# rahulaggarwal965/vslam

Measured on AMD Instinct MI355X. Metric: frame-pairs/sec (extract+match+RANSAC) @1280×720, 2k kp, 4096 hyp; 1/2/4/8 GPU, higher is better.
Workload: dtype u8/f32/f64; 1 GPU; C3: 1280x720, 2000 keypoints, 4096 hypotheses, batch 256 pairs per GPU, SURVEY 8(d) data: rotation + parallax, sub-pixel resampling, 40-45 % outlier matches; pairs_per_gpu=256, batches_in_flight=4

## Files before the change

vslam_amd/build.py:

```python
import os
import subprocess
import sys

HERE = os.path.dirname(os.path.abspath(__file__))
CSRC = os.path.join(HERE, "csrc")
LIB = os.path.join(HERE, "libvslam_amd.so")
SOURCES = ["capi.hip", "match.hip", "ransac_sets.hip", "ransac_solve.hip", "ransac_count.hip", "ransac_prune.hip", "ransac_select.hip", "refit.hip", "refine.hip",
           "kdtree.hip", "gray.hip", "response.hip", "select.hip", "blur.hip",
           "brief.hip", "orb_grid.hip", "pose.hip", "assoc.hip", "map.hip", "world.hip", "resect.hip", "adjust.hip", "render.hip", "multi.hip", "pipeline.hip"]
HEADERS = ["ctx.h", "introselect.h", "image_common.h", "ransac_svd.h", "ransac_residual.h", "ransac_prune_cert.h", "refine_math.h", "resect_math.h", "adjust_math.h", "world_select.h", "world_match.h",
           os.path.join("..", "..", "include", "vslam_amd.h"),
           os.path.join("..", "..", "include", "vslam_resect.h"),
           os.path.join("..", "..", "include", "vslam_adjust.h"),
           os.path.join("..", "..", "include", "vslam_brief_pattern_31.h")]
FLAGS = ["--offload-arch=gfx950", "-O3", "-std=c++17", "-ffp-contract=off", "-fPIC", "-Wall"]
EXTRA_FLAGS = {"response.hip": ["-fno-slp-vectorize"]}
OBJDIR = os.path.join(HERE, "_obj")


EXP_LIB = os.path.join(HERE, "libvslam_amd_exp.so")
EXP_OBJDIR = os.path.join(HERE, "_obj_exp")


def _compile(hipcc, src, verbose, objdir=None, extra=()):
    objdir = objdir or OBJDIR
    obj = os.path.join(objdir, src.replace(".hip", ".o"))
    deps = [os.path.join(CSRC, src)] + [os.path.join(CSRC, h) for h in HEADERS] + [os.path.abspath(__file__)]
    if os.path.exists(obj) and all(os.path.getmtime(d) <= os.path.getmtime(obj) for d in deps):
        return obj, None
    cmd = [hipcc] + FLAGS + list(extra) + EXTRA_FLAGS.get(src, []) + ["-c", "-o", obj, src]
    if verbose:
        print(" ".join(cmd))
    return obj, subprocess.Popen(cmd, cwd=CSRC)


def build(force=False, verbose=False, experiments=False):
    hipcc = os.environ.get("HIPCC", "/opt/rocm/bin/hipcc")
    objdir, lib, extra = (EXP_OBJDIR, EXP_LIB, ("-DVSLAM_EXPERIMENTS",)) if experiments else (OBJDIR, LIB, ())
    return _build(hipcc, objdir, lib, extra, force, verbose)


def _build(hipcc, OBJDIR, LIB, extra, force, verbose):
    os.makedirs(OBJDIR, exist_ok=True)
# ... 45 lines not shown
```

vslam_amd/capi.py:

```python
import ctypes as C
import os

_HERE = os.path.dirname(os.path.abspath(__file__))
LIB_PATH = os.environ.get("VSLAM_AMD_LIB") or os.path.join(_HERE, "libvslam_amd.so")
EXP_LIB_PATH = os.path.join(_HERE, "libvslam_amd_exp.so")

OK = 0
ERRORS = {-1: "VSLAM_ERR_INVALID", -2: "VSLAM_ERR_HIP", -3: "VSLAM_ERR_NO_DEVICE",
          -4: "VSLAM_ERR_CAPACITY", -5: "VSLAM_ERR_DEGENERATE", -6: "VSLAM_ERR_COMM"}

SYMBOLS = [
    "vslam_ctx_create", "vslam_ctx_make_current", "vslam_ctx_destroy", "vslam_ctx_set_stream", "vslam_ctx_set_option", "vslam_ctx_synchronize", "vslam_ctx_wait",
    "vslam_last_error", "vslam_ctx_workspace_bytes", "vslam_version", "vslam_brief_pattern_31", "vslam_dev_alloc", "vslam_dev_free", "vslam_copy_h2d",
    "vslam_copy_d2h", "vslam_debug_stream_copy", "vslam_debug_valu_calib", "vslam_prof_enable", "vslam_prof_reset", "vslam_prof_count", "vslam_prof_get",
    "vslam_match_knn2_ratio", "vslam_ransac_sets", "vslam_ransac_fundamental", "vslam_ransac_solve",
    "vslam_ransac_evaluate", "vslam_refit_fundamental", "vslam_refine_pairs", "vslam_kdtree_build",
    "vslam_kdtree_radius", "vslam_kdtree_nearest", "vslam_kdtree_cell_table", "vslam_extract_features", "vslam_extract_features_grid", "vslam_triangulate_points", "vslam_frontend_pairs_pose", "vslam_pipeline_batches_redone", "vslam_corner_stats", "vslam_bgr2gray", "vslam_min_eigen",
    "vslam_good_features", "vslam_gaussian7", "vslam_orb_describe", "vslam_extract_Rt", "vslam_triangulate", "vslam_associate_map_points", "vslam_reprojection_filter",
    "vslam_match_features",
    "vslam_map_create", "vslam_map_destroy", "vslam_map_reset", "vslam_map_step", "vslam_map_view", "vslam_map_observations",
    "vslam_track_sequences",
    "vslam_world_create", "vslam_world_destroy", "vslam_world_reset", "vslam_world_step", "vslam_world_lift", "vslam_world_view",
    "vslam_map_attach_world", "vslam_world_render",
    "vslam_view_default", "vslam_view_look_at", "vslam_render_points", "vslam_map_render",
# ... 218 lines not shown
        self._check(self.lib.vslam_prof_reset(self.handle))

    def prof_report(self):
        n = self.lib.vslam_prof_count(self.handle)
        if n < 0:
            self._check(n)
        out = {}
        for i in range(n):
            name = C.create_string_buffer(128)
            ms = C.c_double()
            cnt = C.c_int64()
            self._check(self.lib.vslam_prof_get(self.handle, C.c_int(i), name, C.c_int(128), C.byref(ms), C.byref(cnt)))
            out[name.value.decode()] = (ms.value, cnt.value)
        return out

    def debug_detect(self, bgr, max_corners, width=None):
        torch = self.torch
        F, H = bgr.shape[0], bgr.shape[1]
        W = width if width is not None else bgr.shape[2]
        stride = bgr.shape[2] * (bgr.shape[3] if bgr.dim() == 4 else 1)
        xy = torch.zeros((F, max_corners, 2), dtype=torch.float32, device=bgr.device)
        n = torch.zeros((F,), dtype=torch.int32, device=bgr.device)
        self._ready()
        self._check(self.lib.vslam_debug_detect(self.handle, _ptr(bgr), C.c_int(F), C.c_int(W), C.c_int(H), C.c_int(stride),
                                                C.c_int(max_corners), C.c_int(max_corners), _ptr(xy), _ptr(n)))
        return xy, n

    def debug_ransac_prune_x(self, batch, hyp):
        torch = self.torch
        x = torch.zeros((batch, hyp), dtype=torch.int32, device="cuda")
        self._ready()
        self._check(self.lib.vslam_debug_ransac_prune_x(self.handle, _ptr(x), C.c_int(batch), C.c_int(hyp)))
        return x

    def debug_ransac_prune_tile(self, F, xy):
        torch = self.torch
        self._dev(F, torch.float32, "F"); self._dev(xy, torch.float32, "xy")
        assert tuple(F.shape) == (32, 9) and tuple(xy.shape) == (4, 32)
        n = torch.zeros((32, 32), dtype=torch.float32, device=F.device)
        a0 = torch.zeros((32, 32), dtype=torch.float32, device=F.device)
        self._ready()
        self._check(self.lib.vslam_debug_ransac_prune_tile(self.handle, _ptr(F), _ptr(xy), _ptr(n), _ptr(a0)))
        return n, a0

    def debug_valu_calib(self):
        self._check(self.lib.vslam_debug_valu_calib(self.handle))

    def debug_stream_copy(self, src, dst, bytes_per_lane):
        self._check(self.lib.vslam_debug_stream_copy(self.handle, _ptr(src), _ptr(dst), C.c_size_t(src.numel() * src.element_size()),
                                                     C.c_int(bytes_per_lane)))

    def match_knn2_ratio(self, desc1, n1, desc2, n2, want_knn=False):
        torch = self.torch
        B, K, _ = desc1.shape
        self._dev(desc1, torch.uint8, "desc1"); self._dev(desc2, torch.uint8, "desc2")
        self._dev(n1, torch.int32, "n1"); self._dev(n2, torch.int32, "n2")
        pairs = torch.empty((B, K, 2), dtype=torch.int32, device=desc1.device)
        m = torch.empty((B,), dtype=torch.int32, device=desc1.device)
        knn = torch.empty((B, K, 4), dtype=torch.int32, device=desc1.device) if want_knn else None
        self._check(self.lib.vslam_match_knn2_ratio(self.handle, _ptr(desc1), _ptr(n1), _ptr(desc2), _ptr(n2),
                                                    C.c_int(B), C.c_int(K), _ptr(pairs), _ptr(m), _ptr(knn)))
        return (pairs, m, knn) if want_knn else (pairs, m)

    def ransac_sets(self, seeds, m, hyp):
        torch = self.torch
        B = seeds.shape[0]
# ... 937 lines not shown
```

vslam_amd/csrc/ransac_count.hip:

```cpp
#include "ransac_residual.h"

namespace {
using namespace vs_ransac;

constexpr int kCntHyps = 128;
constexpr int kCntWaves = 8;
constexpr int kCntQueue = 320;
constexpr int kCntLdsMatches = 4096;
constexpr int kScreenMatches = 128;
constexpr int kScreenHyps = 128;
constexpr int kRankThreads = 512;
constexpr int kPilotHyps = kRankThreads / 64;
constexpr int kCandMax = 8;
constexpr float kCntTinyDD = 0x1p-120f;
constexpr int kFcmpOGT = 2, kFcmpOLT = 4, kFcmpULT = 12;
constexpr int kCntRec = 12;
typedef __attribute__((address_space(3))) volatile uint32_t cnt_queue_t;
static_assert(VSLAM_MAX_KP <= 65536, "queue words keep the match index in 16 bits");

__host__ __device__ constexpr int cnt_pad(int n) { return (n + 255) & ~255; }
constexpr int kHeadUncertified = -1;
__device__ __forceinline__ float cnt_sum_rel(int adds) { return fmaxf(0x1p-18f, (float)(13 + adds) * 0x1p-24f); }

struct CntBand {
    float lo, hi;
    double beta;
    bool ok;
};
__device__ __forceinline__ CntBand cnt_band(const float *f, float C1, float C2, float threshold) {
    CntBand B;
    bool ok = threshold >= 0x1p-20f && threshold <= 0x1p20f && C1 <= 0x1p20f && C2 <= 0x1p20f;
#pragma unroll
// ... 384 lines not shown
            int p = __popcll(va & ~oa) + __popcll(vb & ~ob);
            int c = __popcll(va & ia) + __popcll(vb & ib);
            if (__builtin_amdgcn_fcmpf(fminf(dd[u].x, dd[u].y), kCntTinyDD, kFcmpULT) != 0ull) {
                p = n0;
                c = 0xFF;
            }
            mine = lane == j + u ? (p | (c << 8)) : mine;
            any_alive = any_alive || p + (m - n0) >= bound_pilots;
        }
        if (!any_alive) continue;
        float v[kU];
#pragma unroll
        for (int u = 0; u < kU; u++) v[u] = (in_a ? g[u].x : 0.f) + (in_b ? g[u].y : 0.f);
        const int z = 0;
        const float k01 = odd1 ? v[1] : v[0], t01 = odd1 ? v[0] : v[1], k23 = odd1 ? v[3] : v[2], t23 = odd1 ? v[2] : v[3];
        const float r01 = k01 + __int_as_float(__builtin_amdgcn_update_dpp(z, __float_as_int(t01), 0xB1, 0xF, 0xF, false));
        const float r23 = k23 + __int_as_float(__builtin_amdgcn_update_dpp(z, __float_as_int(t23), 0xB1, 0xF, 0xF, false));
        const float kk = odd2 ? r23 : r01, tt = odd2 ? r01 : r23;
        float r = kk + __int_as_float(__builtin_amdgcn_update_dpp(z, __float_as_int(tt), 0x4E, 0xF, 0xF, false));
        r += __int_as_float(__builtin_amdgcn_update_dpp(z, __float_as_int(r), 0x124, 0xF, 0xF, false));
        r += __int_as_float(__builtin_amdgcn_update_dpp(z, __float_as_int(r), 0x128, 0xF, 0xF, false));
        r += __shfl_xor(r, 16, 64);
        r += __shfl_xor(r, 32, 64);
        mine_sum = (lane >> 2) == (j >> 2) ? r : mine_sum;
    }
    const int h = hbase + wave * 32 + lane;
    if (lane < 32 && h < hyp) {
        const int c = mine >> 8;
        pot0[(size_t)b * hyp + h] = mine & 0xFF;
        head[(size_t)b * hyp + h] = make_int2(c == 0xFF ? kHeadUncertified : c, __float_as_int(mine_sum));
    }
}

__global__ __launch_bounds__(64 * kCandMax) void ransac_cand_kernel(
    const float *__restrict__ rk, int kp_pad, const int32_t *__restrict__ m_arr, int min_m, int kp_stride, int hyp,
    float threshold, const float *__restrict__ hypF, const int32_t *__restrict__ pot0, int by_sum,
    int32_t *__restrict__ cbound, unsigned long long *__restrict__ sfloor) {
    const int b = blockIdx.x, tid = threadIdx.x, lane = tid & 63;
    const int wave = __builtin_amdgcn_readfirstlane(tid >> 6);
    const int m = min(m_arr[b], kp_stride);
    if (m < min_m) return;
    __shared__ int s_max[kCandMax], s_l0[kCandMax][kCandMax], s_l1[kCandMax][kCandMax], s_n0[kCandMax], s_n1[kCandMax];
    __shared__ int s_cand[kCandMax], s_nc;
    const int32_t *P = pot0 + (size_t)b * hyp;
    int mx = -1;
    for (int i = tid; i < hyp; i += 64 * kCandMax) mx = max(mx, P[i]);
#pragma unroll
    for (int off = 32; off > 0; off >>= 1) mx = max(mx, __shfl_xor(mx, off, 64));
    if (lane == 0) s_max[wave] = mx;
    __syncthreads();
    mx = s_max[0];
    for (int w = 1; w < kCandMax; w++) mx = max(mx, s_max[w]);
    const int per = (hyp + kCandMax - 1) / kCandMax;
    const int lo = min(hyp, wave * per), hi = min(hyp, lo + per);
    int n0 = 0, n1 = 0;
    __shared__ int s_samp[kCandMax][32];
    int nsamp = 0;
    for (int i0 = lo; i0 < hi && ((by_sum && nsamp < 32) || n0 < kCandMax || n1 < kCandMax); i0 += 64) {
        const int i = i0 + lane;
        const int v = i < hi ? P[i] : -2;
        unsigned long long b0 = __ballot(v == mx), b1 = __ballot(v == mx - 1);
        if (by_sum) {
            const int rs = nsamp + __popcll(b0 & ((1ull << lane) - 1ull));
            if (v == mx && rs < 32) s_samp[wave][rs] = i;
            nsamp = min(32, nsamp + (int)__popcll(b0));
        }
        const int r0 = n0 + __popcll(b0 & ((1ull << lane) - 1ull)), r1 = n1 + __popcll(b1 & ((1ull << lane) - 1ull));
        if (v == mx && r0 < kCandMax) s_l0[wave][r0] = i;
        if (v == mx - 1 && r1 < kCandMax) s_l1[wave][r1] = i;
        n0 = min(kCandMax, n0 + __popcll(b0));
        n1 = min(kCandMax, n1 + __popcll(b1));
    }
    if (by_sum && nsamp > 1) {
        const int n128 = min(m, kScreenMatches);
        const float *r = rk + (size_t)b * 4 * kp_pad;
        const float2 x1 = *reinterpret_cast<const float2 *>(r + 2 * lane), y1 = *reinterpret_cast<const float2 *>(r + kp_pad + 2 * lane);
        const float2 x2 = *reinterpret_cast<const float2 *>(r + 2 * kp_pad + 2 * lane), y2 = *reinterpret_cast<const float2 *>(r + 3 * kp_pad + 2 * lane);
        v2f X1, Y1, X2, Y2;
        X1.x = x1.x; X1.y = x1.y; Y1.x = y1.x; Y1.y = y1.y;
        X2.x = x2.x; X2.y = x2.y; Y2.x = y2.x; Y2.y = y2.y;
        float fl[9];
        {
            const int hs = s_samp[wave][lane < nsamp ? lane : 0];
            const float *src = hypF + ((size_t)b * hyp + hs) * 9;
// ... 38 lines not shown
        s_nc = n;
    }
    __syncthreads();
    __shared__ int s_ccount[kCandMax];
    __shared__ double s_csum[kCandMax];
    if (wave < s_nc) {
        const int h = s_cand[wave];
        double esum = 0;
        const int count = cnt_exact_ranked(hypF + ((size_t)b * hyp + h) * 9, rk + (size_t)b * 4 * kp_pad, kp_pad, m, threshold, lane, &esum);
        if (lane == 0) {
            atomicMax(&cbound[b], count);
            s_ccount[wave] = count;
            s_csum[wave] = esum;
        }
    }
    __syncthreads();
    if (tid == 0) {
        int cb = -1;
        for (int k = 0; k < s_nc; k++) cb = max(cb, s_ccount[k]);
        double fl = -INFINITY;
        bool any_nan = false;
        for (int k = 0; k < s_nc; k++)
            if (s_ccount[k] == cb) {
                any_nan = any_nan || !(s_csum[k] == s_csum[k]);
                if (s_csum[k] > fl) fl = s_csum[k];
            }
        const bool valid = cb > 0 && !any_nan && fl > 0 && fl < 0x1p120;
        const float flf = (float)(fl * (1.0 - 0x1p-20));
        const unsigned long long mine = valid ? ((unsigned long long)(uint32_t)cb << 32) | (unsigned long long)__float_as_uint(flf) : 0ull;
        const unsigned long long pilots = sfloor[b];
        sfloor[b] = mine > pilots ? mine : pilots;
    }
}

#ifdef VSLAM_EXPERIMENTS
#define VS_CNT_PAYLOAD_PARAM , int exit_payload
#define VS_CNT_PAYLOAD_ARG , exit_payload
#else
#define VS_CNT_PAYLOAD_PARAM
#define VS_CNT_PAYLOAD_ARG
#endif
template <bool LDS, bool ZERO>
__global__ __launch_bounds__(64 * kCntWaves) __attribute__((amdgpu_waves_per_eu(6, 6))) void ransac_count_kernel(
    const float *__restrict__ rk, int kp_pad, const int32_t *__restrict__ m_arr, int min_m, int kp_stride, int hyp, float threshold,
    const float *__restrict__ hypF, const int32_t *__restrict__ pot0, const int2 *__restrict__ head,
    const float *__restrict__ cmax, int32_t *__restrict__ hyp_count, float *__restrict__ hyp_sum, float *__restrict__ approx,
    int32_t *__restrict__ cbound, const unsigned long long *__restrict__ sfloor VS_CNT_PAYLOAD_PARAM) {
    const int b = blockIdx.y, tid = threadIdx.x, lane = tid & 63;
    const int wave = __builtin_amdgcn_readfirstlane(tid >> 6);
    const int hbase = blockIdx.x * kCntHyps;
    const int nh = min(kCntHyps, hyp - hbase);
    const int m = min(m_arr[b], kp_stride);
    if (m < min_m) return;

    __shared__ __align__(16) float s_rec[kCntHyps * kCntRec];
    __shared__ int s_cnt[kCntHyps];
    __shared__ float s_part[kCntHyps];
    constexpr int kHeadMine = 0x10000, kHeadNoSum = 0x20000;
    __shared__ int s_unk[kCntHyps];
    __shared__ int s_state[kCntHyps];
    __shared__ int s_list[kCntHyps];
    constexpr int kListWaves = kCntHyps / 64;
    static_assert(kCntHyps % 64 == 0 && kListWaves <= kCntWaves, "whole waves find the survivors");
    __shared__ int s_nlist[kListWaves], s_next, s_bound;
    extern __shared__ __align__(16) uint32_t s_dyn[];

// ... 187 lines not shown
        if (st == 1 && my_ok && !s_unk[tid]) {
            const double Sd = (double)S;
            const double rel = (double)cnt_sum_rel(2 * ((m - (ZERO ? 0 : n0) + 255) >> 8) + 9);
            err = (float)((2.02 * my_beta * sqrt((double)m * Sd) + (double)m * my_beta * my_beta + rel * Sd) * (1.0 + 0x1p-20));
        }
        reinterpret_cast<float2 *>(approx)[out] = make_float2(S, err);
    }
}

}

int vs_launch_ransac_count(vslam_ctx *ctx, const float *xy1, const float *xy2, const int32_t *pairs, const int32_t *m,
                           const float *hypF, int batch, int kp_stride, int hyp, float threshold, int32_t *hyp_count,
                           float *hyp_sum, float *approx) {
    const int min_m = ctx->ransac_min_matches;
    int rc;
    int32_t *cbound = nullptr, *pot0 = nullptr;
    float *rk = nullptr, *cmax = nullptr;
    const int kp_pad = cnt_pad(kp_stride);
    if ((rc = vs_arena_get(ctx, "ransac.cbound", sizeof(int32_t) * (size_t)batch, (void **)&cbound))) return rc;
    unsigned long long *sfloor = nullptr;
    if ((rc = vs_arena_get(ctx, "ransac.sfloor", sizeof(unsigned long long) * (size_t)batch, (void **)&sfloor))) return rc;
    static const bool no_sum_rule = VS_EXPERIMENT_ENV("VSLAM_RANSAC_NO_SUM_RULE") != nullptr;
    const bool from_zero = VS_EXPERIMENT_ENV("VSLAM_RANSAC_COUNT_FROM_ZERO") != nullptr;
#ifdef VSLAM_EXPERIMENTS
    const int exit_payload = VS_EXPERIMENT_ENV("VSLAM_RANSAC_COUNT_EXIT_PAYLOAD") != nullptr ? 1 : 0;
#endif
    int2 *head = nullptr;
    if ((rc = vs_arena_get(ctx, "ransac.head", sizeof(int2) * (size_t)batch * hyp, (void **)&head))) return rc;
    const unsigned long long *use_floor = no_sum_rule ? nullptr : sfloor;
    if ((rc = vs_arena_get(ctx, "ransac.pot0", sizeof(int32_t) * (size_t)batch * hyp, (void **)&pot0))) return rc;
    if ((rc = vs_arena_get(ctx, "ransac.rk", sizeof(float) * 4 * (size_t)kp_pad * batch, (void **)&rk))) return rc;
    if ((rc = vs_arena_get(ctx, "ransac.cmax", sizeof(float) * 2 * (size_t)batch, (void **)&cmax))) return rc;
    {
        VsProfScope ps(ctx, "ransac_rank_kernel");
        ransac_rank_kernel<<<batch, kRankThreads, 0, ctx->stream>>>(xy1, xy2, pairs, m, min_m, kp_stride, kp_pad, hyp, threshold, hypF,
                                                                    cbound, rk, cmax, sfloor);
    }
    {
        VsProfScope ps(ctx, "ransac_screen_kernel");
        dim3 grid(vs_div_up(hyp, kScreenHyps), batch);
        ransac_screen_kernel<<<grid, 256, 0, ctx->stream>>>(rk, kp_pad, m, min_m, kp_stride, hyp, threshold, hypF, cmax, cbound, pot0, head);
    }
    {
        VsProfScope ps(ctx, "ransac_cand_kernel");
        ransac_cand_kernel<<<batch, 64 * kCandMax, 0, ctx->stream>>>(rk, kp_pad, m, min_m, kp_stride, hyp, threshold, hypF, pot0,
                                                                     no_sum_rule ? 0 : 1, cbound, sfloor);
    }
    if ((rc = vs_launch_ransac_prune(ctx, rk, kp_pad, m, min_m, kp_stride, hyp, threshold, hypF, cmax, cbound, pot0, batch, kScreenMatches)))
        return rc;
    if (int arc = vs_aux_job_point(ctx, 4)) return arc;
    {
        VsProfScope ps(ctx, "ransac_count_kernel");
        const bool lds = kp_pad <= kCntLdsMatches;
        const size_t dyn = (lds ? sizeof(float) * 4 * (size_t)kp_pad : 0) + sizeof(uint32_t) * kCntQueue * kCntWaves;
        const size_t dyn_max = sizeof(float) * 4 * kCntLdsMatches + sizeof(uint32_t) * kCntQueue * kCntWaves;
        dim3 grid(vs_div_up(hyp, kCntHyps), batch);
#ifdef VSLAM_EXPERIMENTS
        if (from_zero) {
            if (dyn > 32 * 1024 && (rc = vs_allow_dynamic_lds(ctx, ransac_count_kernel<true, true>, "ransac_count_from_zero", dyn_max)))
                return rc;
            if (lds)
                ransac_count_kernel<true, true><<<grid, 64 * kCntWaves, dyn, ctx->stream>>>(
                    rk, kp_pad, m, min_m, kp_stride, hyp, threshold, hypF, pot0, head, cmax, hyp_count, hyp_sum, approx, cbound,
                    use_floor VS_CNT_PAYLOAD_ARG);
            else
                ransac_count_kernel<false, true><<<grid, 64 * kCntWaves, dyn, ctx->stream>>>(
                    rk, kp_pad, m, min_m, kp_stride, hyp, threshold, hypF, pot0, head, cmax, hyp_count, hyp_sum, approx, cbound,
                    use_floor VS_CNT_PAYLOAD_ARG);
            return VSLAM_OK;
        }
#endif
        (void)from_zero;
        if (dyn > 32 * 1024 &&
            (rc = vs_allow_dynamic_lds(ctx, ransac_count_kernel<true, false>, "ransac_count", dyn_max)))
            return rc;
        if (lds)
            ransac_count_kernel<true, false><<<grid, 64 * kCntWaves, dyn, ctx->stream>>>(
                rk, kp_pad, m, min_m, kp_stride, hyp, threshold, hypF, pot0, head, cmax, hyp_count, hyp_sum, approx, cbound,
                    use_floor VS_CNT_PAYLOAD_ARG);
        else
            ransac_count_kernel<false, false><<<grid, 64 * kCntWaves, dyn, ctx->stream>>>(
                rk, kp_pad, m, min_m, kp_stride, hyp, threshold, hypF, pot0, head, cmax, hyp_count, hyp_sum, approx, cbound,
                    use_floor VS_CNT_PAYLOAD_ARG);
    }
    return VSLAM_OK;
}
```

vslam_amd/csrc/ransac_prune.hip:

```cpp
#include "ransac_prune_cert.h"
#include "ransac_residual.h"

namespace {

typedef float v16f __attribute__((ext_vector_type(16)));
constexpr int kPruneWaves = 4;
constexpr int kPruneHyps = 32;
constexpr int kPruneTile = 32;
constexpr int kPruneStep = 2;
constexpr int kPruneOGT = 2;

__host__ __device__ constexpr int prune_row(int r, int half) { return (r & 3) + 8 * (r >> 2) + 4 * half; }

struct PruneA {
    float n[5], d[2];
};
__device__ __forceinline__ PruneA prune_operands(const float *f, bool half) {
    PruneA A;
#pragma unroll
    for (int s = 0; s < 4; s++) A.n[s] = half ? f[2 * s + 1] : f[2 * s];
    A.n[4] = half ? 0.f : f[8];
    A.d[0] = half ? f[1] : f[0];
    A.d[1] = half ? 0.f : f[2];
    return A;
}

__device__ __forceinline__ void prune_tile(const PruneA &A, bool half, float x1, float y1, float x2, float y2, v16f &n, v16f &a0) {
    const float p = x2 * (half ? y1 : x1);
    const float q = y2 * (half ? x1 : y1);
    const float b1 = half ? q : x2, b2 = half ? y2 : q, b3 = half ? y1 : x1, b4 = half ? 0.f : 1.f;
    v16f z;
#pragma unroll
    for (int r = 0; r < 16; r++) z[r] = 0.f;
    n = __builtin_amdgcn_mfma_f32_32x32x2f32(A.n[0], p, z, 0, 0, 0);
    n = __builtin_amdgcn_mfma_f32_32x32x2f32(A.n[1], b1, n, 0, 0, 0);
    n = __builtin_amdgcn_mfma_f32_32x32x2f32(A.n[2], b2, n, 0, 0, 0);
    n = __builtin_amdgcn_mfma_f32_32x32x2f32(A.n[3], b3, n, 0, 0, 0);
    n = __builtin_amdgcn_mfma_f32_32x32x2f32(A.n[4], b4, n, 0, 0, 0);
    a0 = __builtin_amdgcn_mfma_f32_32x32x2f32(A.d[0], b3, z, 0, 0, 0);
    a0 = __builtin_amdgcn_mfma_f32_32x32x2f32(A.d[1], b4, a0, 0, 0, 0);
}

#ifdef VSLAM_EXPERIMENTS
#define VS_PRUNE_X_PARAM , int32_t *__restrict__ x_out
#else
#define VS_PRUNE_X_PARAM
#endif

__global__ __launch_bounds__(64 * kPruneWaves) void ransac_prune_mfma_kernel(
    const float *__restrict__ rk, int kp_pad, const int32_t *__restrict__ m_arr, int min_m, int kp_stride, int hyp, float threshold,
    float splus, const float *__restrict__ hypF, const float *__restrict__ cmax, const int32_t *__restrict__ cbound, int32_t *__restrict__ pot0,
    int n_head, int gate VS_PRUNE_X_PARAM) {
    const int b = blockIdx.y, lane = threadIdx.x & 63, col = lane & 31;
    const bool half = lane >= 32;
    const int wave = __builtin_amdgcn_readfirstlane(threadIdx.x >> 6);
    const int m = min(m_arr[b], kp_stride);
    const int bound = cbound[b];
    if (m < min_m) return;
    const int n0 = min(m, n_head);
    const int hbase = (blockIdx.x * kPruneWaves + wave) * kPruneHyps;
    if (m <= n0 || hbase >= hyp) return;
    if (gate && m - bound + 1 <= n0) return;

    const int h = hbase + col;
    const size_t hi = (size_t)b * hyp + min(h, hyp - 1);
    const int behind = m - n0;
    const int lim = pot0[hi] + behind - bound;
    bool live0 = h < hyp && lim >= 0 && lim < behind;
    if (__ballot(live0) == 0ull) return;
    float f[9];
#pragma unroll
    for (int k = 0; k < 9; k++) f[k] = hypF[hi * 9 + k];
    const float c = pc_margin(f, cmax[2 * b], cmax[2 * b + 1], threshold, splus);
    live0 = live0 && c < INFINITY;
    if (__ballot(live0) == 0ull) return;
    const PruneA A = prune_operands(f, half);
    float cr[16];
#pragma unroll
    for (int r = 0; r < 16; r++) cr[r] = __shfl(c, half ? prune_row(r, 1) : prune_row(r, 0), 64);

    const float *r1 = rk + (size_t)b * 4 * kp_pad, *r2 = r1 + kp_pad, *r3 = r2 + kp_pad, *r4 = r3 + kp_pad;
    int X[kPruneHyps], L[kPruneHyps];
#pragma unroll
    for (int i = 0; i < kPruneHyps; i++) {
        X[i] = 0;
        L[i] = __builtin_amdgcn_readlane(live0 ? lim : -1, i);
    }
    const int end = m;
    for (int base = n0; base < end; base += kPruneStep * kPruneTile) {
        float x1[kPruneStep], y1[kPruneStep], x2[kPruneStep], y2[kPruneStep];
#pragma unroll
        for (int t = 0; t < kPruneStep; t++) {
            const int j = min(base + t * kPruneTile + col, m - 1);
            x1[t] = r1[j];
            y1[t] = r2[j];
            x2[t] = r3[j];
            y2[t] = r4[j];
        }
#pragma unroll
        for (int t = 0; t < kPruneStep; t++) {
            v16f n, a0;
            prune_tile(A, half, x1[t], y1[t], x2[t], y2[t], n, a0);
            const unsigned long long valid = __ballot(base + t * kPruneTile + col < end);
#pragma unroll
            for (int r = 0; r < 16; r++) {
                const unsigned long long miss =
                    __builtin_amdgcn_fcmpf(fabsf(n[r]), fmaf(splus, fabsf(a0[r]), cr[r]), kPruneOGT) & valid;
                X[prune_row(r, 0)] += __popc((uint32_t)miss);
                X[prune_row(r, 1)] += __popc((uint32_t)(miss >> 32));
            }
        }
        int top = -1;
#pragma unroll
        for (int i = 0; i < kPruneHyps; i++) top = max(top, X[i] <= L[i] ? X[i] : -1);
        const int seen = min(base + kPruneStep * kPruneTile, end) - n0;
        if (top < 0 || 2 * top < seen) break;
    }
    int xv = 0;
#pragma unroll
    for (int i = 0; i < kPruneHyps; i++) xv = col == i ? X[i] : xv;
    if (!half && h < hyp) {
        if (live0 && xv > lim) pot0[hi] = -behind - 1;
#ifdef VSLAM_EXPERIMENTS
        if (x_out) x_out[hi] = xv;
#endif
    }
}

#ifdef VSLAM_EXPERIMENTS
__global__ __launch_bounds__(64) void ransac_prune_tile_kernel(const float *__restrict__ F, const float *__restrict__ xy,
                                                               float *__restrict__ n_out, float *__restrict__ a0_out) {
    const int lane = threadIdx.x, col = lane & 31;
    const bool half = lane >= 32;
    float f[9];
#pragma unroll
    for (int k = 0; k < 9; k++) f[k] = F[col * 9 + k];
    const PruneA A = prune_operands(f, half);
    v16f n, a0;
    prune_tile(A, half, xy[col], xy[32 + col], xy[64 + col], xy[96 + col], n, a0);
#pragma unroll
    for (int r = 0; r < 16; r++) {
        const int row = half ? prune_row(r, 1) : prune_row(r, 0);
        n_out[row * 32 + col] = n[r];
        a0_out[row * 32 + col] = a0[r];
    }
}
#endif

}

int vs_launch_ransac_prune(vslam_ctx *ctx, const float *rk, int kp_pad, const int32_t *m, int min_m, int kp_stride, int hyp,
                           float threshold, const float *hypF, const float *cmax, const int32_t *cbound, int32_t *pot0, int batch,
                           int n_head) {
    if (VS_EXPERIMENT_ENV("VSLAM_RANSAC_NO_PRUNE") != nullptr) return VSLAM_OK;
    int gate = 1;
    if (const char *e = VS_EXPERIMENT_ENV("VSLAM_RANSAC_PRUNE_GATE")) gate = atoi(e);
#ifdef VSLAM_EXPERIMENTS
    int32_t *x_out = nullptr;
    if (int rc = vs_arena_get(ctx, "ransac.prune_x", sizeof(int32_t) * (size_t)batch * hyp, (void **)&x_out)) return rc;
    VS_HIP(ctx, hipMemsetAsync(x_out, 0, sizeof(int32_t) * (size_t)batch * hyp, ctx->stream));
#endif
    VsProfScope ps(ctx, "ransac_prune_kernel");
    dim3 grid(vs_div_up(hyp, kPruneWaves * kPruneHyps), batch);
#ifdef VSLAM_EXPERIMENTS
    ransac_prune_mfma_kernel<<<grid, 64 * kPruneWaves, 0, ctx->stream>>>(rk, kp_pad, m, min_m, kp_stride, hyp, threshold, pc_splus(threshold), hypF, cmax,
                                                                         cbound, pot0, n_head, gate, x_out);
#else
    ransac_prune_mfma_kernel<<<grid, 64 * kPruneWaves, 0, ctx->stream>>>(rk, kp_pad, m, min_m, kp_stride, hyp, threshold, pc_splus(threshold), hypF, cmax,
                                                                         cbound, pot0, n_head, gate);
#endif
    return VSLAM_OK;
}

#ifdef VSLAM_EXPERIMENTS
extern "C" {
int vslam_debug_ransac_prune_x(vslam_ctx *ctx, int32_t *d_out, int batch, int hyp) {
    if (!ctx) return VSLAM_ERR_INVALID;
    VS_REQUIRE(ctx, d_out && batch > 0 && hyp > 0 && vs_ptr_bits(d_out) % 4 == 0, VSLAM_ERR_INVALID);
    const size_t bytes = sizeof(int32_t) * (size_t)batch * hyp;
    const auto it = ctx->arena.find("ransac.prune_x");
    VS_REQUIRE(ctx, it != ctx->arena.end() && it->second.bytes >= bytes, VSLAM_ERR_INVALID);
    VS_HIP(ctx, hipMemcpyAsync(d_out, it->second.ptr, bytes, hipMemcpyDeviceToDevice, ctx->stream));
    return VSLAM_OK;
}
int vslam_debug_ransac_prune_tile(vslam_ctx *ctx, const float *d_F, const float *d_xy, float *d_n, float *d_a0) {
    if (!ctx) return VSLAM_ERR_INVALID;
    VS_REQUIRE(ctx, d_F && d_xy && d_n && d_a0 && vs_ptr_bits(d_F, d_xy, d_n, d_a0) % 4 == 0, VSLAM_ERR_INVALID);
    ransac_prune_tile_kernel<<<1, 64, 0, ctx->stream>>>(d_F, d_xy, d_n, d_a0);
    return VSLAM_OK;
}
}
#endif
```

vslam_amd/csrc/ransac_residual.h:

```cpp
#pragma once

#include "ctx.h"

namespace vs_ransac {

struct ResidualF {
    float f[9];
    double ft[6];
};
__device__ __forceinline__ void residual_prepare(ResidualF &R) {
    R.ft[0] = (double)R.f[0];
    R.ft[1] = (double)R.f[3];
    R.ft[2] = (double)R.f[6];
    R.ft[3] = (double)R.f[1];
    R.ft[4] = (double)R.f[4];
    R.ft[5] = (double)R.f[7];
}
__device__ __forceinline__ float residual_e(const ResidualF &R, const float4 c, const double dx2, const double dy2) {
    const float x1 = c.x, y1 = c.y, x2 = c.z, y2 = c.w;
    const float a0 = R.f[0] * x1 + R.f[1] * y1 + R.f[2];
    const float a1 = R.f[3] * x1 + R.f[4] * y1 + R.f[5];
    const float a2 = R.f[6] * x1 + R.f[7] * y1 + R.f[8];
    const float t0 = (float)(__builtin_fma(R.ft[1], dy2, R.ft[0] * dx2) + R.ft[2]);
    const float t1 = (float)(__builtin_fma(R.ft[4], dy2, R.ft[3] * dx2) + R.ft[5]);
    const float n = (x2 * a0 + y2 * a1) + a2;
    const float q = (n * n) / (a0 * a0);
    return ((q + a1 * a1) + t0 * t0) + t1 * t1;
}

typedef float v2f __attribute__((ext_vector_type(2)));
__device__ __forceinline__ v2f residual_e2(const ResidualF &R, const v2f x1, const v2f y1, const v2f x2, const v2f y2,
                                           const double2 da, const double2 db) {
    const v2f a0 = (R.f[0] * x1 + R.f[1] * y1) + R.f[2];
    const v2f a1 = (R.f[3] * x1 + R.f[4] * y1) + R.f[5];
    const v2f a2 = (R.f[6] * x1 + R.f[7] * y1) + R.f[8];
    v2f t0, t1;
    t0.x = (float)(__builtin_fma(R.ft[1], da.y, R.ft[0] * da.x) + R.ft[2]);
    t0.y = (float)(__builtin_fma(R.ft[1], db.y, R.ft[0] * db.x) + R.ft[2]);
    t1.x = (float)(__builtin_fma(R.ft[4], da.y, R.ft[3] * da.x) + R.ft[5]);
    t1.y = (float)(__builtin_fma(R.ft[4], db.y, R.ft[3] * db.x) + R.ft[5]);
    const v2f n = (x2 * a0 + y2 * a1) + a2;
    const v2f nn = n * n, dd = a0 * a0;
    v2f q;
    q.x = nn.x / dd.x;
    q.y = nn.y / dd.y;
    return ((q + a1 * a1) + t0 * t0) + t1 * t1;
}

}

int vs_launch_ransac_count(vslam_ctx *ctx, const float *xy1, const float *xy2, const int32_t *pairs, const int32_t *m,
                           const float *hypF, int batch, int kp_stride, int hyp, float threshold, int32_t *hyp_count,
                           float *hyp_sum, float *approx);

int vs_launch_ransac_prune(vslam_ctx *ctx, const float *rk, int kp_pad, const int32_t *m, int min_m, int kp_stride, int hyp,
                           float threshold, const float *hypF, const float *cmax, const int32_t *cbound, int32_t *pot0, int batch,
                           int n_head);
```

Before: 100,600 frame-pairs/s.

## Bucket hypotheses by screen score so prune waves group similar early-exit work

The candidate kernel now also builds a per-pair counting-sort permutation of hypotheses keyed by their clamped pot0 score, written as uint16 or int32 indices. The prune kernel reads hypotheses through this order, so each 32-hypothesis wave holds hypotheses with similar bounds and can exit its tile walk together instead of being held by one long-running member. The prune grid is also flattened onto an XCD-aware item/block mapping. This adds histogram, scan and scatter work plus an extra arena buffer in the candidate kernel, and an indirect gather in prune.

```diff
diff --git a/vslam_amd/build.py b/vslam_amd/build.py
--- a/vslam_amd/build.py
+++ b/vslam_amd/build.py
@@ -8,7 +8,7 @@
 SOURCES = ["capi.hip", "match.hip", "ransac_sets.hip", "ransac_solve.hip", "ransac_count.hip", "ransac_prune.hip", "ransac_select.hip", "refit.hip", "refine.hip",
            "kdtree.hip", "gray.hip", "response.hip", "select.hip", "blur.hip",
            "brief.hip", "orb_grid.hip", "pose.hip", "assoc.hip", "map.hip", "world.hip", "resect.hip", "adjust.hip", "render.hip", "multi.hip", "pipeline.hip"]
-HEADERS = ["ctx.h", "introselect.h", "image_common.h", "ransac_svd.h", "ransac_residual.h", "ransac_prune_cert.h", "refine_math.h", "resect_math.h", "adjust_math.h", "world_select.h", "world_match.h",
+HEADERS = ["ctx.h", "introselect.h", "image_common.h", "ransac_svd.h", "ransac_residual.h", "ransac_prune_cert.h", "ransac_order.h", "refine_math.h", "resect_math.h", "adjust_math.h", "world_select.h", "world_match.h",
            os.path.join("..", "..", "include", "vslam_amd.h"),
            os.path.join("..", "..", "include", "vslam_resect.h"),
            os.path.join("..", "..", "include", "vslam_adjust.h"),
diff --git a/vslam_amd/capi.py b/vslam_amd/capi.py
--- a/vslam_amd/capi.py
+++ b/vslam_amd/capi.py
@@ -274,6 +274,44 @@
         self._ready()
         self._check(self.lib.vslam_debug_ransac_prune_x(self.handle, _ptr(x), C.c_int(batch), C.c_int(hyp)))
         return x
+
+    def debug_ransac_prune_tiles(self, batch, hyp):
+        torch = self.torch
+        t = torch.zeros((batch, (hyp + 31) // 32), dtype=torch.int32, device="cuda")
+        self._ready()
+        self._check(self.lib.vslam_debug_ransac_prune_tiles(self.handle, _ptr(t), C.c_int(batch), C.c_int(hyp)))
+        return t
+
+    def _order_tensor(self, batch, hyp):
+        torch = self.torch
+        return torch.zeros((batch, hyp), dtype=torch.int16 if hyp <= 65536 else torch.int32, device="cuda")
+
+    @staticmethod
+    def order_numpy(order):
+        a = order.cpu().numpy()
+        return (a.view("uint16") if a.dtype.itemsize == 2 else a).astype("int64")
+
+    def debug_ransac_prune_order(self, batch, hyp):
+        o = self._order_tensor(batch, hyp)
+        self._ready()
+        self._check(self.lib.vslam_debug_ransac_prune_order(self.handle, _ptr(o), C.c_int(batch), C.c_int(hyp)))
+        return o
+
+    def debug_ransac_pot0(self, batch, hyp):
+        torch = self.torch
+        p = torch.zeros((batch, hyp), dtype=torch.int32, device="cuda")
+        self._ready()
+        self._check(self.lib.vslam_debug_ransac_pot0(self.handle, _ptr(p), C.c_int(batch), C.c_int(hyp)))
+        return p
+
+    def debug_ransac_order(self, pot0):
+        torch = self.torch
+        self._dev(pot0, torch.int32, "pot0")
+        batch, hyp = pot0.shape
+        o = self._order_tensor(batch, hyp)
+        self._ready()
+        self._check(self.lib.vslam_debug_ransac_order(self.handle, _ptr(pot0), C.c_int(batch), C.c_int(hyp), _ptr(o)))
+        return o
 
     def debug_ransac_prune_tile(self, F, xy):
         torch = self.torch
diff --git a/vslam_amd/csrc/ransac_count.hip b/vslam_amd/csrc/ransac_count.hip
--- a/vslam_amd/csrc/ransac_count.hip
+++ b/vslam_amd/csrc/ransac_count.hip
@@ -1,3 +1,4 @@
+#include "ransac_order.h"
 #include "ransac_residual.h"
 
 namespace {
@@ -448,24 +449,106 @@
     }
 }
 
+__device__ __forceinline__ void cand_write_order(const int32_t *__restrict__ P, int hyp, void *__restrict__ order_pair, bool wide,
+                                                 int (*s_hist)[kOrderKeys], int *s_tot, int *s_max, int tid, int lane, int wave) {
+    for (int i = tid; i < kOrderWaves * kOrderKeys; i += 64 * kOrderWaves) (&s_hist[0][0])[i] = 0;
+    __syncthreads();
+    int lo, hi;
+    order_share(hyp, wave, lo, hi);
+    constexpr int kU = 8;
+    const bool once = hi - lo <= 64 * kU;
+    int raw[kU], mx = -1;
+    for (int c0 = lo; c0 < hi; c0 += 64 * kU) {
+#pragma unroll
+        for (int u = 0; u < kU; u++) raw[u] = c0 + 64 * u + lane < hi ? P[c0 + 64 * u + lane] : -1;
+#pragma unroll
+        for (int u = 0; u < kU; u++) {
+            mx = max(mx, raw[u]);
+            if (c0 + 64 * u + lane < hi) atomicAdd(&s_hist[wave][order_key(raw[u])], 1);
+        }
+    }
+#pragma unroll
+    for (int off = 32; off > 0; off >>= 1) mx = max(mx, __shfl_xor(mx, off, 64));
+    if (lane == 0) s_max[wave] = mx;
+    __syncthreads();
+    if (tid < kOrderKeys) {
+        int run = 0;
+        for (int w = 0; w < kOrderWaves; w++) {
+            const int t = s_hist[w][tid];
+            s_hist[w][tid] = run;
+            run += t;
+        }
+        s_tot[tid] = run;
+    }
+    __syncthreads();
+    if (wave == 0) {
+        static_assert(kOrderKeys <= 3 * 64, "three keys per lane");
+        int v[3], s = 0;
+#pragma unroll
+        for (int j = 0; j < 3; j++) {
+            v[j] = 3 * lane + j < kOrderKeys ? s_tot[3 * lane + j] : 0;
+            s += v[j];
+        }
+        int incl = s;
+#pragma unroll
+        for (int off = 1; off < 64; off <<= 1) {
+            const int t = __shfl_up(incl, off, 64);
+            if (lane >= off) incl += t;
+        }
+        int run = incl - s;
+#pragma unroll
+        for (int j = 0; j < 3; j++) {
+            if (3 * lane + j < kOrderKeys) s_tot[3 * lane + j] = run;
+            run += v[j];
+        }
+    }
+    __syncthreads();
+    volatile int *wb = s_hist[wave];
+    const unsigned long long below = (1ull << lane) - 1ull;
+    for (int c0 = lo; c0 < hi; c0 += 64 * kU) {
+        if (!once) {
+#pragma unroll
+            for (int u = 0; u < kU; u++) raw[u] = c0 + 64 * u + lane < hi ? P[c0 + 64 * u + lane] : -1;
+        }
+#pragma unroll
+        for (int u = 0; u < kU; u++) {
+            if (c0 + 64 * u >= hi) break;
+            const int i = c0 + 64 * u + lane;
+            const int key = i < hi ? order_key(raw[u]) : kOrderKeys;
+            unsigned long long same = ~0ull;
+#pragma unroll
+            for (int bit = 0; bit < 8; bit++) {
+                const unsigned long long set = __ballot((key >> bit) & 1);
+                same &= ((key >> bit) & 1) ? set : ~set;
+            }
+            if (i < hi) {
+                const int rank = __popcll(same & below), n = __popcll(same);
+                const int at = wb[key];
+                const int pos = s_tot[key] + at + rank;
+                if (wide) reinterpret_cast<int32_t *>(order_pair)[pos] = i;
+                else reinterpret_cast<uint16_t *>(order_pair)[pos] = (uint16_t)i;
+                if (rank == n - 1) wb[key] = at + n;
+            }
+        }
+    }
+}
+
 __global__ __launch_bounds__(64 * kCandMax) void ransac_cand_kernel(
     const float *__restrict__ rk, int kp_pad, const int32_t *__restrict__ m_arr, int min_m, int kp_stride, int hyp,
     float threshold, const float *__restrict__ hypF, const int32_t *__restrict__ pot0, int by_sum,
-    int32_t *__restrict__ cbound, unsigned long long *__restrict__ sfloor) {
+    int32_t *__restrict__ cbound, unsigned long long *__restrict__ sfloor, void *__restrict__ order) {
     const int b = blockIdx.x, tid = threadIdx.x, lane = tid & 63;
     const int wave = __builtin_amdgcn_readfirstlane(tid >> 6);
     const int m = min(m_arr[b], kp_stride);
     if (m < min_m) return;
     __shared__ int s_max[kCandMax], s_l0[kCandMax][kCandMax], s_l1[kCandMax][kCandMax], s_n0[kCandMax], s_n1[kCandMax];
     __shared__ int s_cand[kCandMax], s_nc;
+    __shared__ int s_ohist[kOrderWaves][kOrderKeys], s_otot[kOrderKeys];
+    static_assert(kOrderWaves == kCandMax && kOrderKeyMax == kScreenMatches, "ransac_order.h restates this kernel's shape");
     const int32_t *P = pot0 + (size_t)b * hyp;
-    int mx = -1;
-    for (int i = tid; i < hyp; i += 64 * kCandMax) mx = max(mx, P[i]);
-#pragma unroll
-    for (int off = 32; off > 0; off >>= 1) mx = max(mx, __shfl_xor(mx, off, 64));
-    if (lane == 0) s_max[wave] = mx;
-    __syncthreads();
-    mx = s_max[0];
+    cand_write_order(P, hyp, reinterpret_cast<char *>(order) + (size_t)b * order_bytes(hyp), order_wide(hyp), s_ohist, s_otot, s_max, tid, lane,
+                     wave);
+    int mx = s_max[0];
     for (int w = 1; w < kCandMax; w++) mx = max(mx, s_max[w]);
     const int per = (hyp + kCandMax - 1) / kCandMax;
     const int lo = min(hyp, wave * per), hi = min(hyp, lo + per);
@@ -570,6 +653,15 @@
         sfloor[b] = mine > pilots ? mine : pilots;
     }
 }
+
+#ifdef VSLAM_EXPERIMENTS
+__global__ __launch_bounds__(64 * kOrderWaves) void ransac_order_kernel(const int32_t *__restrict__ pot0, int hyp, void *__restrict__ order) {
+    const int b = blockIdx.x, tid = threadIdx.x;
+    __shared__ int s_ohist[kOrderWaves][kOrderKeys], s_otot[kOrderKeys], s_max[kOrderWaves];
+    cand_write_order(pot0 + (size_t)b * hyp, hyp, reinterpret_cast<char *>(order) + (size_t)b * order_bytes(hyp), order_wide(hyp), s_ohist,
+                     s_otot, s_max, tid, tid & 63, __builtin_amdgcn_readfirstlane(tid >> 6));
+}
+#endif
 
 #ifdef VSLAM_EXPERIMENTS
 #define VS_CNT_PAYLOAD_PARAM , int exit_payload
@@ -823,6 +915,8 @@
     if ((rc = vs_arena_get(ctx, "ransac.pot0", sizeof(int32_t) * (size_t)batch * hyp, (void **)&pot0))) return rc;
     if ((rc = vs_arena_get(ctx, "ransac.rk", sizeof(float) * 4 * (size_t)kp_pad * batch, (void **)&rk))) return rc;
     if ((rc = vs_arena_get(ctx, "ransac.cmax", sizeof(float) * 2 * (size_t)batch, (void **)&cmax))) return rc;
+    void *order = nullptr;
+    if ((rc = vs_arena_get(ctx, "ransac.order", order_bytes(hyp) * (size_t)batch, &order))) return rc;
     {
         VsProfScope ps(ctx, "ransac_rank_kernel");
         ransac_rank_kernel<<<batch, kRankThreads, 0, ctx->stream>>>(xy1, xy2, pairs, m, min_m, kp_stride, kp_pad, hyp, threshold, hypF,
@@ -836,9 +930,9 @@
     {
         VsProfScope ps(ctx, "ransac_cand_kernel");
         ransac_cand_kernel<<<batch, 64 * kCandMax, 0, ctx->stream>>>(rk, kp_pad, m, min_m, kp_stride, hyp, threshold, hypF, pot0,
-                                                                     no_sum_rule ? 0 : 1, cbound, sfloor);
-    }
-    if ((rc = vs_launch_ransac_prune(ctx, rk, kp_pad, m, min_m, kp_stride, hyp, threshold, hypF, cmax, cbound, pot0, batch, kScreenMatches)))
+                                                                     no_sum_rule ? 0 : 1, cbound, sfloor, order);
+    }
+    if ((rc = vs_launch_ransac_prune(ctx, rk, kp_pad, m, min_m, kp_stride, hyp, threshold, hypF, cmax, cbound, pot0, order, batch, kScreenMatches)))
         return rc;
     if (int arc = vs_aux_job_point(ctx, 4)) return arc;
     {
@@ -877,3 +971,33 @@
     }
     return VSLAM_OK;
 }
+
+#ifdef VSLAM_EXPERIMENTS
+namespace {
+int debug_arena_copy(vslam_ctx *ctx, const char *name, void *d_out, size_t bytes) {
+    const auto it = ctx->arena.find(name);
+    VS_REQUIRE(ctx, it != ctx->arena.end() && it->second.bytes >= bytes, VSLAM_ERR_INVALID);
+    VS_HIP(ctx, hipMemcpyAsync(d_out, it->second.ptr, bytes, hipMemcpyDeviceToDevice, ctx->stream));
+    return VSLAM_OK;
+}
+}
+
+extern "C" {
+int vslam_debug_ransac_order(vslam_ctx *ctx, const int32_t *d_pot0, int batch, int hyp, void *d_order) {
+    if (!ctx) return VSLAM_ERR_INVALID;
+    VS_REQUIRE(ctx, d_pot0 && d_order && batch > 0 && hyp > 0 && vs_ptr_bits(d_pot0, d_order) % 4 == 0, VSLAM_ERR_INVALID);
+    ransac_order_kernel<<<batch, 64 * kOrderWaves, 0, ctx->stream>>>(d_pot0, hyp, d_order);
+    return VSLAM_OK;
+}
+int vslam_debug_ransac_prune_order(vslam_ctx *ctx, void *d_out, int batch, int hyp) {
+    if (!ctx) return VSLAM_ERR_INVALID;
+    VS_REQUIRE(ctx, d_out && batch > 0 && hyp > 0 && vs_ptr_bits(d_out) % 4 == 0, VSLAM_ERR_INVALID);
+    return debug_arena_copy(ctx, "ransac.order", d_out, order_bytes(hyp) * (size_t)batch);
+}
+int vslam_debug_ransac_pot0(vslam_ctx *ctx, int32_t *d_out, int batch, int hyp) {
+    if (!ctx) return VSLAM_ERR_INVALID;
+    VS_REQUIRE(ctx, d_out && batch > 0 && hyp > 0 && vs_ptr_bits(d_out) % 4 == 0, VSLAM_ERR_INVALID);
+    return debug_arena_copy(ctx, "ransac.pot0", d_out, sizeof(int32_t) * (size_t)batch * hyp);
+}
+}
+#endif
diff --git a/vslam_amd/csrc/ransac_order.h b/vslam_amd/csrc/ransac_order.h
--- /dev/null
+++ b/vslam_amd/csrc/ransac_order.h
@@ -0,0 +1,50 @@
+#pragma once
+
+#include <cstddef>
+#include <cstdint>
+
+#if defined(__HIPCC__)
+#define PO_HD __host__ __device__ inline
+#else
+#define PO_HD inline
+#endif
+
+constexpr int kOrderKeyMax = 128;
+constexpr int kOrderKeys = kOrderKeyMax + 2;
+constexpr int kOrderWaves = 8;
+constexpr int kOrderNarrowMax = 65536;
+
+PO_HD int order_key(int pot0) { return pot0 < 0 ? kOrderKeyMax + 1 : (pot0 > kOrderKeyMax ? kOrderKeyMax : pot0); }
+PO_HD bool order_wide(int hyp) { return hyp > kOrderNarrowMax; }
+PO_HD size_t order_bytes(int hyp) { return (size_t)hyp * (order_wide(hyp) ? 4 : 2); }
+
+PO_HD void order_share(int hyp, int w, int &lo, int &hi) {
+    const int per = (hyp + kOrderWaves - 1) / kOrderWaves;
+    lo = w * per < hyp ? w * per : hyp;
+    hi = lo + per < hyp ? lo + per : hyp;
+}
+
+PO_HD void order_base(const int (*hist)[kOrderKeys], int (*base)[kOrderKeys]) {
+    int run = 0;
+    for (int k = 0; k < kOrderKeys; k++)
+        for (int w = 0; w < kOrderWaves; w++) {
+            base[w][k] = run;
+            run += hist[w][k];
+        }
+}
+
+inline void order_host(const int32_t *pot0, int hyp, uint32_t *order) {
+    int hist[kOrderWaves][kOrderKeys], base[kOrderWaves][kOrderKeys];
+    for (int w = 0; w < kOrderWaves; w++) {
+        for (int k = 0; k < kOrderKeys; k++) hist[w][k] = 0;
+        int lo, hi;
+        order_share(hyp, w, lo, hi);
+        for (int i = lo; i < hi; i++) hist[w][order_key(pot0[i])]++;
+    }
+    order_base(hist, base);
+    for (int w = 0; w < kOrderWaves; w++) {
+        int lo, hi;
+        order_share(hyp, w, lo, hi);
+        for (int i = lo; i < hi; i++) order[base[w][order_key(pot0[i])]++] = (uint32_t)i;
+    }
+}
diff --git a/vslam_amd/csrc/ransac_prune.hip b/vslam_amd/csrc/ransac_prune.hip
--- a/vslam_amd/csrc/ransac_prune.hip
+++ b/vslam_amd/csrc/ransac_prune.hip
@@ -1,3 +1,4 @@
+#include "ransac_order.h"
 #include "ransac_prune_cert.h"
 #include "ransac_residual.h"
 
@@ -42,31 +43,39 @@
 }
 
 #ifdef VSLAM_EXPERIMENTS
-#define VS_PRUNE_X_PARAM , int32_t *__restrict__ x_out
+#define VS_PRUNE_X_PARAM , int32_t *__restrict__ x_out, int32_t *__restrict__ tiles_out
 #else
 #define VS_PRUNE_X_PARAM
 #endif
 
+template <bool WIDE>
 __global__ __launch_bounds__(64 * kPruneWaves) void ransac_prune_mfma_kernel(
     const float *__restrict__ rk, int kp_pad, const int32_t *__restrict__ m_arr, int min_m, int kp_stride, int hyp, float threshold,
     float splus, const float *__restrict__ hypF, const float *__restrict__ cmax, const int32_t *__restrict__ cbound, int32_t *__restrict__ pot0,
-    int n_head, int gate VS_PRUNE_X_PARAM) {
-    const int b = blockIdx.y, lane = threadIdx.x & 63, col = lane & 31;
+    const void *__restrict__ order, int n_head, int gate, int batch, int per_pair VS_PRUNE_X_PARAM) {
+    const int lane = threadIdx.x & 63, col = lane & 31;
     const bool half = lane >= 32;
     const int wave = __builtin_amdgcn_readfirstlane(threadIdx.x >> 6);
+    int b, blk;
+    vs_xcd_item_block(blockIdx.x, per_pair, b, blk);
+    if (b >= batch) return;
+    const int hbase = (blk * kPruneWaves + wave) * kPruneHyps;
+    const bool inside = hbase + col < hyp;
+    const size_t at = (size_t)b * hyp + min(hbase + col, hyp - 1);
+    int h = WIDE ? __hip_atomic_load(reinterpret_cast<const int32_t *>(order) + at, __ATOMIC_RELAXED, __HIP_MEMORY_SCOPE_WAVEFRONT)
+                 : (int)__hip_atomic_load(reinterpret_cast<const uint16_t *>(order) + at, __ATOMIC_RELAXED, __HIP_MEMORY_SCOPE_WAVEFRONT);
     const int m = min(m_arr[b], kp_stride);
     const int bound = cbound[b];
     if (m < min_m) return;
     const int n0 = min(m, n_head);
-    const int hbase = (blockIdx.x * kPruneWaves + wave) * kPruneHyps;
     if (m <= n0 || hbase >= hyp) return;
     if (gate && m - bound + 1 <= n0) return;
 
-    const int h = hbase + col;
-    const size_t hi = (size_t)b * hyp + min(h, hyp - 1);
+    h = (int)min((unsigned)h, (unsigned)(hyp - 1));
+    const size_t hi = (size_t)b * hyp + h;
     const int behind = m - n0;
     const int lim = pot0[hi] + behind - bound;
-    bool live0 = h < hyp && lim >= 0 && lim < behind;
+    bool live0 = inside && lim >= 0 && lim < behind;
     if (__ballot(live0) == 0ull) return;
     float f[9];
 #pragma unroll
@@ -87,6 +96,9 @@
         L[i] = __builtin_amdgcn_readlane(live0 ? lim : -1, i);
     }
     const int end = m;
+#ifdef VSLAM_EXPERIMENTS
+    int walked = 0;
+#endif
     for (int base = n0; base < end; base += kPruneStep * kPruneTile) {
         float x1[kPruneStep], y1[kPruneStep], x2[kPruneStep], y2[kPruneStep];
 #pragma unroll
@@ -114,20 +126,32 @@
 #pragma unroll
         for (int i = 0; i < kPruneHyps; i++) top = max(top, X[i] <= L[i] ? X[i] : -1);
         const int seen = min(base + kPruneStep * kPruneTile, end) - n0;
+#ifdef VSLAM_EXPERIMENTS
+        walked = (seen + kPruneTile - 1) / kPruneTile;
+#endif
         if (top < 0 || 2 * top < seen) break;
     }
     int xv = 0;
 #pragma unroll
     for (int i = 0; i < kPruneHyps; i++) xv = col == i ? X[i] : xv;
-    if (!half && h < hyp) {
+    if (!half && inside) {
         if (live0 && xv > lim) pot0[hi] = -behind - 1;
 #ifdef VSLAM_EXPERIMENTS
         if (x_out) x_out[hi] = xv;
 #endif
     }
-}
-
-#ifdef VSLAM_EXPERIMENTS
+#ifdef VSLAM_EXPERIMENTS
+    if (tiles_out && lane == 0) tiles_out[(size_t)b * ((hyp + kPruneHyps - 1) / kPruneHyps) + hbase / kPruneHyps] = walked;
+#endif
+}
+
+#ifdef VSLAM_EXPERIMENTS
+__global__ void ransac_order_identity_kernel(void *__restrict__ order, int wide, int hyp, size_t total) {
+    const size_t i = (size_t)blockIdx.x * blockDim.x + threadIdx.x;
+    if (i >= total) return;
+    if (wide) reinterpret_cast<int32_t *>(order)[i] = (int32_t)(i % hyp);
+    else reinterpret_cast<uint16_t *>(order)[i] = (uint16_t)(i % hyp);
+}
 __global__ __launch_bounds__(64) void ransac_prune_tile_kernel(const float *__restrict__ F, const float *__restrict__ xy,
                                                                float *__restrict__ n_out, float *__restrict__ a0_out) {
     const int lane = threadIdx.x, col = lane & 31;
@@ -150,25 +174,40 @@
 }
 
 int vs_launch_ransac_prune(vslam_ctx *ctx, const float *rk, int kp_pad, const int32_t *m, int min_m, int kp_stride, int hyp,
-                           float threshold, const float *hypF, const float *cmax, const int32_t *cbound, int32_t *pot0, int batch,
-                           int n_head) {
+                           float threshold, const float *hypF, const float *cmax, const int32_t *cbound, int32_t *pot0,
+                           void *order, int batch, int n_head) {
     if (VS_EXPERIMENT_ENV("VSLAM_RANSAC_NO_PRUNE") != nullptr) return VSLAM_OK;
     int gate = 1;
     if (const char *e = VS_EXPERIMENT_ENV("VSLAM_RANSAC_PRUNE_GATE")) gate = atoi(e);
+    const int wide = order_wide(hyp) ? 1 : 0;
 #ifdef VSLAM_EXPERIMENTS
     int32_t *x_out = nullptr;
     if (int rc = vs_arena_get(ctx, "ransac.prune_x", sizeof(int32_t) * (size_t)batch * hyp, (void **)&x_out)) return rc;
     VS_HIP(ctx, hipMemsetAsync(x_out, 0, sizeof(int32_t) * (size_t)batch * hyp, ctx->stream));
+    int32_t *tiles_out = nullptr;
+    const size_t tiles_bytes = sizeof(int32_t) * (size_t)batch * vs_div_up(hyp, kPruneHyps);
+    if (int rc = vs_arena_get(ctx, "ransac.prune_tiles", tiles_bytes, (void **)&tiles_out)) return rc;
+    VS_HIP(ctx, hipMemsetAsync(tiles_out, 0, tiles_bytes, ctx->stream));
+    if (const char *e = VS_EXPERIMENT_ENV("VSLAM_RANSAC_PRUNE_ORDER"))
+        if (atoi(e) == 0) {
+            const size_t total = (size_t)batch * hyp;
+            ransac_order_identity_kernel<<<(unsigned)((total + 255) / 256), 256, 0, ctx->stream>>>(order, wide, hyp, total);
+        }
 #endif
     VsProfScope ps(ctx, "ransac_prune_kernel");
-    dim3 grid(vs_div_up(hyp, kPruneWaves * kPruneHyps), batch);
-#ifdef VSLAM_EXPERIMENTS
-    ransac_prune_mfma_kernel<<<grid, 64 * kPruneWaves, 0, ctx->stream>>>(rk, kp_pad, m, min_m, kp_stride, hyp, threshold, pc_splus(threshold), hypF, cmax,
-                                                                         cbound, pot0, n_head, gate, x_out);
+    const int per_pair = vs_div_up(hyp, kPruneWaves * kPruneHyps);
+    const int grid = vs_xcd_grid(batch, per_pair);
+#ifdef VSLAM_EXPERIMENTS
+#define VS_PRUNE_X_ARG , x_out, tiles_out
 #else
-    ransac_prune_mfma_kernel<<<grid, 64 * kPruneWaves, 0, ctx->stream>>>(rk, kp_pad, m, min_m, kp_stride, hyp, threshold, pc_splus(threshold), hypF, cmax,
-                                                                         cbound, pot0, n_head, gate);
-#endif
+#define VS_PRUNE_X_ARG
+#endif
+    if (wide)
+        ransac_prune_mfma_kernel<true><<<grid, 64 * kPruneWaves, 0, ctx->stream>>>(rk, kp_pad, m, min_m, kp_stride, hyp, threshold, pc_splus(threshold),
+                                                                                   hypF, cmax, cbound, pot0, order, n_head, gate, batch, per_pair VS_PRUNE_X_ARG);
+    else
+        ransac_prune_mfma_kernel<false><<<grid, 64 * kPruneWaves, 0, ctx->stream>>>(rk, kp_pad, m, min_m, kp_stride, hyp, threshold, pc_splus(threshold),
+                                                                                    hypF, cmax, cbound, pot0, order, n_head, gate, batch, per_pair VS_PRUNE_X_ARG);
     return VSLAM_OK;
 }
 
@@ -183,6 +222,15 @@
     VS_HIP(ctx, hipMemcpyAsync(d_out, it->second.ptr, bytes, hipMemcpyDeviceToDevice, ctx->stream));
     return VSLAM_OK;
 }
+int vslam_debug_ransac_prune_tiles(vslam_ctx *ctx, int32_t *d_out, int batch, int hyp) {
+    if (!ctx) return VSLAM_ERR_INVALID;
+    VS_REQUIRE(ctx, d_out && batch > 0 && hyp > 0 && vs_ptr_bits(d_out) % 4 == 0, VSLAM_ERR_INVALID);
+    const size_t bytes = sizeof(int32_t) * (size_t)batch * vs_div_up(hyp, kPruneHyps);
+    const auto it = ctx->arena.find("ransac.prune_tiles");
+    VS_REQUIRE(ctx, it != ctx->arena.end() && it->second.bytes >= bytes, VSLAM_ERR_INVALID);
+    VS_HIP(ctx, hipMemcpyAsync(d_out, it->second.ptr, bytes, hipMemcpyDeviceToDevice, ctx->stream));
+    return VSLAM_OK;
+}
 int vslam_debug_ransac_prune_tile(vslam_ctx *ctx, const float *d_F, const float *d_xy, float *d_n, float *d_a0) {
     if (!ctx) return VSLAM_ERR_INVALID;
     VS_REQUIRE(ctx, d_F && d_xy && d_n && d_a0 && vs_ptr_bits(d_F, d_xy, d_n, d_a0) % 4 == 0, VSLAM_ERR_INVALID);
diff --git a/vslam_amd/csrc/ransac_residual.h b/vslam_amd/csrc/ransac_residual.h
--- a/vslam_amd/csrc/ransac_residual.h
+++ b/vslam_amd/csrc/ransac_residual.h
@@ -54,5 +54,5 @@
                            float *hyp_sum, float *approx);
 
 int vs_launch_ransac_prune(vslam_ctx *ctx, const float *rk, int kp_pad, const int32_t *m, int min_m, int kp_stride, int hyp,
-                           float threshold, const float *hypF, const float *cmax, const int32_t *cbound, int32_t *pot0, int batch,
-                           int n_head);
+                           float threshold, const float *hypF, const float *cmax, const int32_t *cbound, int32_t *pot0, void *order,
+                           int batch, int n_head);
```

Result: no change. 101,000 frame-pairs/s (median of 2 runs) (+0.3%).
